# ehsan886/DBA_mod

Measured on AMD Instinct MI355X. Metric: FL rounds/sec + backdoor ASR & main-task acc, ResNet-18 CIFAR-10 100 clients, higher is better.
Workload: dtype fp32

## Files before the change

### csrc/kernels/xconv_fwd.hip

```cpp
#include "xhalo.hpp"

namespace xg {
SplitPolicy& split_policy() {
  static SplitPolicy p;
  return p;
}
}

namespace {

template <int W, int IMGS, int BN, int WM, int WN, bool PRE>
__global__ __launch_bounds__(256) void ximg_kernel(const XArgs a) {
  constexpr int P = 2, NT = 256;
  constexpr int PW = W + 2, PI = PW * PW, PP = IMGS * PI;
  constexpr int CC = 32, CH = CC / 8, Q4 = CC / 4;
  constexpr int PATCH = PP * CH;
  constexpr int BM = IMGS * W * W;
  constexpr int TM = BM / WM, TN = BN / WN, MI = TM / 32, NJ = TN / 32;
  static_assert(WM * WN == NT / 64 && MI >= 1 && NJ >= 1 && BM == 128, "tiling");
  constexpr int RPT = NT / 8;
  static_assert(BN % RPT == 0, "weight rows");
  constexpr int RB = BN / RPT, BPL = BN * 4;
  __shared__ __attribute__((aligned(16))) uint4 patch[P * PATCH];
  __shared__ __attribute__((aligned(16))) uint4 bring[2 * P * BPL];
// ... 76 lines not shown
#pragma unroll
  for (int i = 0; i < MI; ++i)
#pragma unroll
    for (int j = 0; j < NJ; ++j)
#pragma unroll
      for (int r = 0; r < 16; ++r) acc[i][j][r] = 0.f;

  int apix[MI], arow[MI];
#pragma unroll
  for (int i = 0; i < MI; ++i) {
    const int m = wm * TM + i * 32 + fr;
    const int im = m / (W * W), rem = m - im * (W * W);
    apix[i] = im * PI + (rem / W) * PW + rem % W;
    arow[i] = rem / W;
  }
  auto mma = [&](int t, int buf, int stn) __attribute__((always_inline)) {
    const int tap = t % 9, ti = tap / 3, tj = tap - ti * 3;
    const int toff = ti * PW + tj;
    const uint4* L = bring + buf * P * BPL;
    sfor<2>([&](auto KK) __attribute__((always_inline)) {
      const int ch = decltype(KK)::value * 2 + hf;
      uint4 af[P][MI], bfr[P][NJ];
#pragma unroll
      for (int i = 0; i < MI; ++i) {
        const int pp = apix[i] + toff;
        const int o = pp * CH + (ch ^ ((arow[i] + ti) & 3));
#pragma unroll
        for (int p = 0; p < P; ++p) af[p][i] = patch[p * PATCH + o];
      }
#pragma unroll
      for (int j = 0; j < NJ; ++j) {
        const int n = wn * TN + j * 32 + fr;
        const int o = n * 4 + (ch ^ ((n >> 2) & 3));
#pragma unroll
        for (int p = 0; p < P; ++p) bfr[p][j] = L[p * BPL + o];
      }
      mma_half<MI, NJ, P, true, RB, decltype(KK)::value>(af, bfr, acc, [&](int q) __attribute__((always_inline)) {
        lput_q(buf ^ 1, stn, q);
        gq(t + 3, stn, q);
      });
    });
  };
  auto step = [&](int t, int buf, int stn) __attribute__((always_inline)) {
    const int c = t / 9;
    mma(t, buf, stn);
    __syncthreads();
    if (t - 9 * c == 8 && c + 1 < NC) {
#pragma unroll
      for (int u = 0; u < NE; ++u) ppiece(u, hs.ma);
      if (c + 2 < NC) pload(c + 2);
      __syncthreads();
    }
  };

  hs.init(amax_read(a.amax_src, a.amax_src_ld, g), amax_read(a.amax_w, a.amax_w_ld, slot));
#pragma unroll
  for (int q = 0; q < RB; ++q) {
    gq(0, 0, q);
    gq(1, 1, q);
  }
  pload(0);
#pragma unroll
  for (int u = 0; u < NE; ++u) ppiece(u, hs.ma);
  if (NC > 1) pload(1);
#pragma unroll
  for (int q = 0; q < RB; ++q) {
    lput_q(0, 0, q);
    gq(2, 0, q);
  }
  __syncthreads();
  int t = 0;
  for (; t + 1 < NK; t += 2) {
    step(t, 0, 1);
    step(t + 1, 1, 0);
  }
  if (t < NK) step(t, 0, 1);
  hs.finish(acc);

  float* out = a.out + (long long)g * a.out_gstride;
  const float* bias = a.bias ? a.bias + (long long)slot * a.b_sstride : nullptr;
  const float* res = a.res ? a.res + (long long)g * a.out_gstride : nullptr;
  float vmax = 0.f;
#pragma unroll
  for (int j = 0; j < NJ; ++j) {
    const int n = n0 + wn * TN + j * 32 + fr;
    if (n >= a.Ncol) continue;
    const float bv = bias ? bias[n] : 0.f;
#pragma unroll
    for (int i = 0; i < MI; ++i)
#pragma unroll
      for (int r = 0; r < 16; ++r) {
        const int m = wm * TM + i * 32 + (r & 3) + 8 * (r >> 2) + 4 * hf;
        if (img0 + m / (W * W) >= nv) continue;
        const long long o = (long long)(img0 * W * W + m) * a.Ncol + n;
        float v = acc[i][j][r];
        if (bias) v += bv;
        if (res) v += res[o];
        if (a.relu) v = fmaxf(v, 0.f);
        vmax = fmaxf(vmax, fabsf(v));
        out[o] = v;
      }
  }
  if (a.amax_out) amax_fold(a.amax_out, a.amax_out_ld, g, vmax);
}

template <int W, int IMGS, int BN>
__global__ __launch_bounds__(256) void ximg2_kernel(const XArgs a) {
  constexpr int P = 2, NT = 256;
  constexpr int PW = W + 2, PI = PW * PW, PP = IMGS * PI;
  constexpr int CC = 32, CH = CC / 8, Q4 = CC / 4;
  constexpr int PATCH = PP * CH;
  constexpr int BM = IMGS * W * W;
  constexpr int WN = BN / 32, WM = (NT / 64) / WN, TM = BM / WM, MI = TM / 32;
  static_assert(WM * WN == NT / 64 && MI >= 1 && BM == 128, "tiling");
  extern __shared__ __attribute__((aligned(16))) uint4 ximg2_patch[];

  const int g = blockIdx.y;
  const int tn = blockIdx.x % a.tiles_n, tm = blockIdx.x / a.tiles_n;
  const int img0 = tm * IMGS, n0 = tn * BN;
  const int nv = min(valid_rows(a.nvalid, g, a.N), a.N);
  if (img0 >= nv) return;
  const int slot = a.wsel ? a.wsel[g] : g;
  const int Cs = a.Cs, NC = Cs / CC, NK = 9 * NC;
  const float* __restrict__ src = a.src + (long long)g * a.src_gstride;
  const int tid = threadIdx.x, lane = tid & 63, wid = tid >> 6;
  const int wm = wid / WN, wn = wid % WN;
  const int fr = lane & 31, hf = lane >> 5;

  constexpr int NE = (PP * Q4 + NT - 1) / NT;
  static_assert(NE <= 9, "one patch piece per k-step");
  float4 pv[NE];
  const __amdgpu_buffer_rsrc_t rA = rsrc(src, (long long)a.N * W * W * Cs * 4);
  auto pload1 = [&](int u, int cc) __attribute__((always_inline)) {
    const int e = tid + NT * u;
    const int pp = e / Q4, q = e - pp * Q4;
    const int im = pp / PI, rem = pp - im * PI;
    const int h = rem / PW - 1, w = rem % PW - 1, img = img0 + im;
    const bool ok = e < PP * Q4 && cc < NC && img < nv && (unsigned)h < (unsigned)W && (unsigned)w < (unsigned)W;
    pv[u] = bload4(rA, ok ? (((img * W + h) * W + w) * Cs + cc * CC + q * 4) * 4 : kOOB);
  };
  HScale hs;
  auto ppiece = [&](int u, int buf) __attribute__((always_inline)) {
    const int e = tid + NT * u;
    if (NT * (u + 1) > PP * Q4 && e >= PP * Q4) return;
    const int pp = e / Q4, q = e - pp * Q4;
    const int prow = (pp % PI) / PW;
    uint2 sp[P];
    split4h(pv[u].x, pv[u].y, pv[u].z, pv[u].w, hs.ma, sp);
    const int o = pp * CH + ((q >> 1) ^ (prow & 3));
#pragma unroll
    for (int p = 0; p < P; ++p) ((uint2*)&ximg2_patch[(buf * P + p) * PATCH + o])[q & 1] = sp[p];
  };

  const __amdgpu_buffer_rsrc_t rF = rsrc(a.wf + (long long)slot * a.wf_sstride, (long long)a.Ncol * 9 * Cs * 4);
  const int wbase = ((n0 >> 5) + wn) * NK * 4096 + lane * 16;
  uint4 wb[3][4];
  auto gw = [&](int t, int s, int f) __attribute__((always_inline)) {
    wb[s][f] = __builtin_bit_cast(uint4, bload4(rF, t < NK ? wbase + t * 4096 + f * 1024 : kOOB));
  };

  f32x16_t acc[MI][1];
#pragma unroll
  for (int i = 0; i < MI; ++i)
#pragma unroll
    for (int r = 0; r < 16; ++r) acc[i][0][r] = 0.f;

  int apix[MI], arow[MI];
#pragma unroll
  for (int i = 0; i < MI; ++i) {
    const int m = wm * TM + i * 32 + fr;
    const int im = m / (W * W), rem = m - im * (W * W);
    apix[i] = im * PI + (rem / W) * PW + rem % W;
    arow[i] = rem / W;
  }

  hs.init(amax_read(a.amax_src, a.amax_src_ld, g), amax_read(a.amax_w, a.amax_w_ld, slot));
#pragma unroll
  for (int f = 0; f < 4; ++f) {
    gw(0, 0, f);
    gw(1, 1, f);
  }
#pragma unroll
  for (int u = 0; u < NE; ++u) pload1(u, 0);
#pragma unroll
  for (int u = 0; u < NE; ++u) {
    ppiece(u, 0);
    pload1(u, 1);
  }
  __syncthreads();
  for (int c = 0; c < NC; ++c) {
    const uint4* L = ximg2_patch + (c & 1) * P * PATCH;
    const bool more = c + 1 < NC;
    sfor<9>([&](auto TAP) __attribute__((always_inline)) {
      constexpr int tap = decltype(TAP)::value, ti = tap / 3, tj = tap - ti * 3;
      constexpr int toff = ti * PW + tj, s = tap % 3, s2 = (tap + 2) % 3;
      constexpr int u = tap - (9 - NE);
      constexpr int NQ = u >= 0 ? 5 : 4;
      const int t = c * 9 + tap;
      __builtin_amdgcn_sched_barrier(0x786);
      sfor<2>([&](auto KK) __attribute__((always_inline)) {
        constexpr int kk = decltype(KK)::value;
        const int ch = kk * 2 + hf;
        uint4 af[P][MI], bfr[P][1];
#pragma unroll
        for (int i = 0; i < MI; ++i) {
          const int o = (apix[i] + toff) * CH + (ch ^ ((arow[i] + ti) & 3));
#pragma unroll
          for (int p = 0; p < P; ++p) af[p][i] = L[p * PATCH + o];
        }
#pragma unroll
        for (int p = 0; p < P; ++p) bfr[p][0] = wb[s][kk * 2 + p];
        mma_half<MI, 1, P, true, NQ, kk>(af, bfr, acc, [&](int q) __attribute__((always_inline)) {
          if (q < 4) {
            gw(t + 2, s2, q);
          } else if constexpr (u >= 0) {
            if (more) ppiece(u, (c + 1) & 1);
            pload1(u, c + 2);
          }
        });
      });
    });
    __syncthreads();
  }
  hs.finish(acc);

  float* out = a.out + (long long)g * a.out_gstride;
  const float* bias = a.bias ? a.bias + (long long)slot * a.b_sstride : nullptr;
  const float* res = a.res ? a.res + (long long)g * a.out_gstride : nullptr;
  float vmax = 0.f;
  const int n = n0 + wn * 32 + fr;
  if (n < a.Ncol) {
    const float bv = bias ? bias[n] : 0.f;
#pragma unroll
    for (int i = 0; i < MI; ++i)
#pragma unroll
      for (int r = 0; r < 16; ++r) {
        const int m = wm * TM + i * 32 + (r & 3) + 8 * (r >> 2) + 4 * hf;
        if (img0 + m / (W * W) >= nv) continue;
        const long long o = (long long)(img0 * W * W + m) * a.Ncol + n;
        float v = acc[i][0][r];
        if (bias) v += bv;
        if (res) v += res[o];
        if (a.relu) v = fmaxf(v, 0.f);
        vmax = fmaxf(vmax, fabsf(v));
        out[o] = v;
      }
  }
  if (a.amax_out) amax_fold(a.amax_out, a.amax_out_ld, g, vmax);
}

template <int W, int IMGS, int BN, int WM, int WN>
int ximg_go(const XArgs& a, int G, hipStream_t st) {
  XArgs b = a;
  b.tiles_n = ceil_div(a.Ncol, BN);
  const dim3 grid((unsigned)(ceil_div(a.N, IMGS) * b.tiles_n), G, 1);
  if (a.wp) hipLaunchKernelGGL((ximg_kernel<W, IMGS, BN, WM, WN, true>), grid, dim3(256), 0, st, b);
  else hipLaunchKernelGGL((ximg_kernel<W, IMGS, BN, WM, WN, false>), grid, dim3(256), 0, st, b);
  DBA_LAUNCH_CHECK();
}
template <int W, int IMGS, int BN>
int ximg2_go(const XArgs& a, int G, hipStream_t st) {
  constexpr int PATCH = IMGS * (W + 2) * (W + 2) * 4;
  constexpr int LDS = 2 * 2 * PATCH * (int)sizeof(uint4);
  static unsigned long long attr_set = 0ull;
  int dev = 0;
  if (hipGetDevice(&dev) != hipSuccess || dev < 0 || dev >= 64) return -100;
  if (!(attr_set >> dev & 1ull)) {
    if (hipFuncSetAttribute((const void*)ximg2_kernel<W, IMGS, BN>, hipFuncAttributeMaxDynamicSharedMemorySize,
                            LDS) != hipSuccess)
      return -100;
    attr_set |= 1ull << dev;
  }
  XArgs b = a;
  b.tiles_n = ceil_div(a.Ncol, BN);
  const dim3 grid((unsigned)(ceil_div(a.N, IMGS) * b.tiles_n), G, 1);
  hipLaunchKernelGGL((ximg2_kernel<W, IMGS, BN>), grid, dim3(256), LDS, st, b);
  DBA_LAUNCH_CHECK();
}
int& ximg_on() {
  static int on = 1;
  return on;
}
int ximg_try(const XArgs& a, int G, int KH, int KW, hipStream_t st) {
  const XClass& c = a.cls[0];
  if (!ximg_on() || KH != 3 || KW != 3 || a.sp != 1 || a.os != 1 || a.dsg != 1 || a.splitk != 1 || c.nI != 3 ||
      c.nJ != 3 || c.bh != -1 || c.bw != -1)
    return -100;
  if (a.Hs != a.Ho || a.Ws != a.Wo || a.Ho != a.Wo || a.Cs % 32 != 0 || a.Ncol % 32 != 0) return -100;
  if (a.bf.mode || a.lz_coef) return -100;
  if (!aligned16(a.src) || a.src_gstride % 4 || !aligned16(a.w) || a.w_sstride % 4) return -100;
  if (a.wp && (((uintptr_t)a.wp & 15) || a.wp_sstride % 8)) return -100;
  if (a.sc_src) return -100;
  if (ximg_on() == 1 && a.wp && a.wf && !((uintptr_t)a.wf & 15) && a.wf_sstride % 8 == 0) {
    int rc = -100;
    if (a.Wo == 8) rc = a.Ncol >= 128 ? ximg2_go<8, 2, 128>(a, G, st) : ximg2_go<8, 2, 64>(a, G, st);
    if (a.Wo == 4) rc = a.Ncol >= 128 ? ximg2_go<4, 8, 128>(a, G, st) : ximg2_go<4, 8, 64>(a, G, st);
    if (rc != -100) return rc;
  }
  if (a.Wo == 8) return a.Ncol >= 128 ? ximg_go<8, 2, 128, 2, 2>(a, G, st) : ximg_go<8, 2, 64, 2, 2>(a, G, st);
  if (a.Wo == 4) return a.Ncol >= 128 ? ximg_go<4, 8, 128, 2, 2>(a, G, st) : ximg_go<4, 8, 64, 2, 2>(a, G, st);
  return -100;
}

}

DBA_EXPORT int dba_xsplit_policy(int target, int min_k, int max_s, int kslab_max, int dgrad_ks) {
  SplitPolicy& p = split_policy();
  if (dgrad_ks >= 0) p.dgrad_ks = dgrad_ks;
  if (target > 0) p.target = target;
  if (min_k > 0) p.min_k = min_k;
  if (max_s > 0) p.max_s = std::min(max_s, kSkMax);
  if (kslab_max > 0) p.kslab_max = kslab_max;
  return 0;
}

DBA_EXPORT int dba_ximg_set(int on) {
  const int prev = ximg_on();
  if (on >= 0) ximg_on() = on;
  return prev;
}


DBA_EXPORT long long dba_xconv_ws_floats(int G, int N, int Ho, int Wo, int Cin, int Cout, int KH, int KW) {
  const long long M = (long long)N * Ho * Wo;
  const int s = xsplitk(M, G, Cout, KH * KW * Cin);
  return s > 1 ? (long long)s * G * M * Cout : 0;
}


DBA_EXPORT long long dba_xconv_sk_ints(int G, int N, int Ho, int Wo, int Cin, int Cout, int KH, int KW) {
  const long long M = (long long)N * Ho * Wo;
  const int s = xsplitk(M, G, Cout, KH * KW * Cin);
  const long long n = s > 1 ? xconv_sk_count(M, Cout, G, 1, s) : 0;
  return (n > 0 && sk_ok((const int*)1, n, M, Cout, G, 1, s)) ? n : 0;
}


DBA_EXPORT int dba_xconv_fwd(const float* x, long long x_gstride, const float* w, long long w_sstride,
                             const int* wsel, const float* bias, long long b_sstride, const float* res, float* out,
                             long long out_gstride, const int* nvalid, int G, int N, int H, int W, int Cin, int Ho,
                             int Wo, int Cout, int KH, int KW, int stride, int pad, int relu, const int* amax_x,
                             int amax_x_ld, const int* amax_w, int amax_w_ld, int* amax_out, int amax_out_ld,
                             const uint16_t* wp, long long wp_sstride, const uint16_t* wf, long long wf_sstride,
                             float* ws, long long ws_floats, int* sk_cnt,
                             long long sk_cnt_n, const void* bnf, const float* lz_coef, int lz_relu,
                             void* stream) {
  hipStream_t st = (hipStream_t)stream;
  if ((long long)N * H * W * Cin >= (1LL << 29)) return -103;
  const long long M = (long long)N * Ho * Wo;
  const int K = KH * KW * Cin;
  const int vec = (Cin % 4 == 0 && aligned16(x) && aligned16(w) && x_gstride % 4 == 0 && w_sstride % 4 == 0) ? 4 : 1;
  XArgs a{};
  a.src = x; a.src_gstride = x_gstride; a.w = w; a.w_sstride = w_sstride; a.wsel = wsel;
  a.bias = bias; a.b_sstride = b_sstride; a.res = res; a.out = out; a.out_gstride = out_gstride;
  a.nvalid = nvalid; a.N = N; a.Hs = H; a.Ws = W; a.Cs = Cin; a.Ncol = Cout; a.Ho = Ho; a.Wo = Wo;
  a.sp = stride; a.os = 1; a.dsg = 1; a.relu = relu; a.splitk = 1;
  a.amax_src = amax_x; a.amax_w = amax_w; a.amax_out = amax_out;
  a.amax_src_ld = amax_x_ld; a.amax_w_ld = amax_w_ld; a.amax_out_ld = amax_out_ld;
  a.wp = wp; a.wp_sstride = wp_sstride; a.wf = wf; a.wf_sstride = wf_sstride;
  a.cls[0] = XClass{KH, KW, -pad, -pad, 0, 0, Ho, Wo, 0};
  if (!amax_x || !amax_w) return -109;
  if (bnf) {
    a.bf = *(const BnFuse*)bnf;
    if (a.bf.mode != 1 || bias || res || relu || (Cout & 3) || a.bf.C != Cout) return -108;
  }
  if (lz_coef) {
    if (wp || vec < 4 || Cin > 512) return -108;
    a.lz_coef = lz_coef; a.lz_relu = lz_relu;
  }
  auto fin = [&](int rc) { return (rc == 0 && a.bf.mode) ? bnx_finalize_go(a.bf, nvalid, G, N, Ho * Wo, st) : rc; };
  if (stride == 1) {
    int rc = ximg_try(a, G, KH, KW, st);
    if (rc == -100) rc = xhalo_try(a, G, KH, KW, st);
    if (rc != -100) return fin(rc);
  }
  const int s = xsplitk(M, G, Cout, K);
  const bool ws_ok = s > 1 && ws != nullptr && ws_floats >= (long long)s * G * M * Cout;
  if (s > 1 && !(ws_ok && sk_ok(sk_cnt, sk_cnt_n, M, Cout, G, 1, s))) {
    XArgs b = a;
    b.kslab = s;
    const int rc = xconv_ks(b, M, G, vec, st);
    if (rc != -100) return fin(rc);
  }
  if (ws_ok && sk_ok(sk_cnt, sk_cnt_n, M, Cout, G, 1, s)) {
    XArgs b = a;
    b.splitk = s;
    b.zstride = (long long)G * M * Cout;
    b.sk_ws = ws; b.sk_gstride = M * Cout; b.sk_cnt = sk_cnt;
    return fin(xconv_dispatch(b, M, G, 1, vec, st));
  }
  if (ws_ok) {
    XArgs b = a;
    b.splitk = s;
    b.out = ws;
    b.out_gstride = M * Cout;
    b.zstride = (long long)G * M * Cout;
    const int rc = xconv_dispatch(b, M, G, 1, vec, st);
    if (rc != 0) return rc;
    if (a.bf.mode)
      return bnx_tile_go(a.bf, nullptr, out, out_gstride, nvalid, G, N, Ho * Wo, nullptr, 0.f, ws, s, b.zstride,
                         nullptr, st);
    const long long per = M * Cout;
    const dim3 grid((unsigned)std::max(1LL, std::min(1024LL, (per + 255) / 256)), G);
    hipLaunchKernelGGL(xsplitk_reduce_kernel, grid, dim3(256), 0, st, (const float*)ws, s, b.zstride, per, nvalid, N,
                       Ho * Wo, Cout, bias, b_sstride, wsel, res, relu, out, amax_out, amax_out_ld);
    DBA_LAUNCH_CHECK();
  }
  return fin(xconv_dispatch(a, M, G, 1, vec, st));
}


DBA_EXPORT int dba_xdown_fwd(const float* a_, long long a_gstride, const float* w2, long long w2_sstride,
                             const uint16_t* w2p, long long w2p_sstride, const int* wsel, const float* b2,
                             long long b_sstride, const float* x2, long long x2_gstride, const uint16_t* wscp,
                             long long wscp_sstride, const float* bsc, long long bsc_sstride, float* out,
                             long long out_gstride, const int* nvalid, int G, int N, int Ho, int Wo, int C, int H2,
                             int W2, int C2, const int* amax_a, int amax_a_ld, const int* amax_w2, int amax_w2_ld,
                             const int* amax_x2, int amax_x2_ld, const int* amax_wsc, int amax_wsc_ld, int* amax_out,
                             int amax_out_ld, void* stream) {
  if (!amax_a || !amax_w2 || !amax_x2 || !amax_wsc || !w2p || !wscp) return -109;
  if ((H2 - 1) / 2 + 1 != Ho || (W2 - 1) / 2 + 1 != Wo || (long long)N * H2 * W2 * C2 >= (1LL << 29) ||
      (long long)N * Ho * Wo * C >= (1LL << 29))
    return -103;
  XArgs a{};
  a.src = a_; a.src_gstride = a_gstride; a.w = w2; a.w_sstride = w2_sstride; a.wsel = wsel;
  a.bias = b2; a.b_sstride = b_sstride; a.res = nullptr; a.out = out; a.out_gstride = out_gstride;
  a.nvalid = nvalid; a.N = N; a.Hs = Ho; a.Ws = Wo; a.Cs = C; a.Ncol = C; a.Ho = Ho; a.Wo = Wo;
  a.sp = 1; a.os = 1; a.dsg = 1; a.relu = 1; a.splitk = 1;
  a.amax_src = amax_a; a.amax_w = amax_w2; a.amax_out = amax_out;
  a.amax_src_ld = amax_a_ld; a.amax_w_ld = amax_w2_ld; a.amax_out_ld = amax_out_ld;
  a.wp = w2p; a.wp_sstride = w2p_sstride;
  a.sc_src = x2; a.sc_gstride = x2_gstride; a.sc_H = H2; a.sc_W = W2; a.sc_C = C2;
  a.sc_wp = wscp; a.sc_wp_sstride = wscp_sstride;
  a.sc_amax_src = amax_x2; a.sc_amax_src_ld = amax_x2_ld; a.sc_amax_w = amax_wsc; a.sc_amax_w_ld = amax_wsc_ld;
  a.sc_bias = bsc; a.sc_b_sstride = bsc_sstride;
  a.cls[0] = XClass{3, 3, -1, -1, 0, 0, Ho, Wo, 0};
  return xhalo_try(a, G, 3, 3, (hipStream_t)stream);
}
```

### dba_mod_amd/ops/hip.py

```python
from __future__ import annotations

import contextlib
import ctypes
import os
from typing import Optional, Sequence, Tuple

import torch

from . import bnstate as bs
from . import build

Tensor = torch.Tensor
_F32 = torch.float32

if not os.path.exists(build.kernels_path()):
    raise ImportError(f"HIP kernel library missing: {build.kernels_path()} — run "
                      f"`python -m dba_mod_amd.ops.build` (or __graft_entry__.build())")
_L = ctypes.CDLL(build.kernels_path())

_P = ctypes.c_void_p
_I = ctypes.c_int
_LL = ctypes.c_longlong
_F = ctypes.c_float
_U = ctypes.c_uint
_D = ctypes.c_double

_SIGS = {
    "dba_gather_images": [_P, _P, _P, _P, _P, _P, _I, _P, _P, _I, _P, _I, _I, _I, _I, _I, _P],
    "dba_gather_rows": [_P, _P, _P, _P, _P, _I, _P, _P, _I, _P, _I, _P, _I, _I, _I, _P],
    "dba_xcolsum": [_P, _LL, _I, _P, _I, _I, _I, _P, _LL, _P, _P],
    "dba_xcolsum_part_doubles": [_I, _I, _I, _I],
    "dba_amax_segments": [_P, _LL, _P, _I, _I, _P, _I, _P],
    "dba_bn_fold": [_P, _LL, _P, _P, _P, _P, _P, _LL, _F, _P, _P, _I, _I, _I, _I, _P, _I, _P],
    "dba_relu_mask_bwd": [_P, _P, _P, _LL, _I, _P],
    "dba_maxpool": [_P, _P, _P, _LL, _I, _I, _I, _I, _I, _I, _I, _I, _I, _P],
    "dba_maxpool_bwd": [_P, _P, _P, _LL, _I, _I, _I, _I, _I, _I, _I, _I, _I, _P],
    "dba_avgpool": [_P, _P, _LL, _I, _I, _I, _P],
    "dba_avgpool_bwd": [_P, _P, _LL, _I, _I, _I, _P],
    "dba_dropout": [_P, _P, _I, _P, _U, _F, _LL, _I, _P],
    "dba_softmax_xent": [_P, _P, _I, _I, _I, _I, _P, _P, _P, _P, _LL, _P, _I, _P, _I, _P, _P, _P],
    "dba_softmax_xent_part_doubles": [_I, _I],
    "dba_xent_r5_set": [_I],
    "dba_head_train": [_P, _LL, _I, _I, _I, _I, _P, _LL, _P, _LL, _I, _P, _P, _P, _P, _P, _P, _LL, _P, _LL, _P, _P,
                       _P, _P, _LL, _P, _I, _I, _P],
    "dba_head_part_doubles": [_I, _I],
    "dba_sgd_step": [_P, _LL, _P, _P, _P, _P, _P, _F, _F, _P, _I, _I, _P],
    "dba_scale_from_base": [_P, _P, _F, _P, _LL, _P],
    "dba_add_noise_scaled": [_P, _P, _LL, _F, _F, _U, _I, _I, _P],
    "dba_delta_sum": [_P, _LL, _I, _P, _LL, _P, _P],
    "dba_sqdist_blocks": [_LL],
    "dba_gram_chunks": [_I],
    "dba_sq_dists": [_P, _LL, _P, _I, _LL, _P, _P, _P],
    "dba_weighted_sum": [_P, _LL, _P, _I, _P, _LL, _I, _P],
    "dba_weighted_sum_fixed": [_P, _LL, _P, _I, _P, _LL, _D, _P],
    "dba_gram": [_P, _LL, _I, _I, _P, _P, _P],
    "dba_delta_stats_blocks": [_LL],
    "dba_delta_stats": [_P, _LL, _I, _P, _LL, _P, _P, _P, _P, _P],
    "dba_clipped_delta_sum_fixed": [_P, _LL, _I, _P, _P, _P, _LL, _D, _P],
    "dba_clipped_delta_sum": [_P, _LL, _I, _P, _P, _P, _LL, _P],
    "dba_dist_loss_grad": [_P, _LL, _P, _LL, _P, _LL, _I, _P, _P, _F, _P, _P, _P],
    "dba_ximg_set": [_I],
    "dba_xwgrad_halo_set": [_I],
    "dba_xconv_ws_floats": [_I] * 8,
    "dba_xconv_fwd": [_P, _LL, _P, _LL, _P, _P, _LL, _P, _P, _LL, _P] + [_I] * 13 + [_P, _I] * 3 + [_P, _LL] * 3
    + [_P, _LL, _P, _P, _I, _P],
    "dba_xconv_sk_ints": [_I] * 8,
    "dba_xconv_dgrad": [_P, _LL, _P, _LL, _P, _P, _P, _LL, _P] + [_I] * 12 + [_P, _I] * 2 + [_P, _LL] * 3 + [_P, _P],
    "dba_xsplit_w": [_P, _LL, _LL, _I, _P, _I, _P, _P],
    "dba_amax": [_P, _LL, _LL, _P, _LL, _I, _P, _I, _P],
    "dba_xtranspose": [_P, _I, _I, _LL, _P, _P],
    "dba_xwgrad_ws_floats": [_I] * 8 + [_P],
    "dba_xwgrad_stem_ws_floats": [_I] * 6,
    "dba_xsplit_policy": [_I] * 5,
    "dba_xsplit_w_batch": [_P, _I, _I, _P],
    "dba_xfrag_w_batch": [_P, _I, _I, _P],
    "dba_bn_fold_batch": [_P, _I, _I, _F, _P],
    "dba_xwgrad": [_P, _LL, _P, _LL, _P, _LL, _P] + [_I] * 12 + [_P, _I] * 2 + [_P, _LL, _I] + [_P, _I, _P],
    "dba_bnx_rows": [_P, _P, _P, _LL, _P, _I, _I, _I, _P, _F, _P],
    "dba_bnx_apply": [_P, _P, _P, _P, _P, _I, _I, _P, _LL, _P, _I, _I, _I, _I, _P, _I, _P],
    "dba_bnfuse_size": [],
    "dba_xwgrad_stem": [_P, _LL, _P, _P, _P, _LL, _P, _P, _I, _I, _I, _I, _P],
    "dba_bnx_dy": [_P, _P, _P, _P, _LL, _P, _I, _I, _I, _I, _P, _I, _P],
    "dba_xwgrad_reduce_batch": [_P, _I, _I, _LL, _P],
    "dba_xblock_fwd": [_P, _LL, _P, _LL, _P, _P, _P, _LL, _P, _P, _LL, _P] + [_I] * 6
    + [_P, _I, _P, _P, _I, _P, _I, _P],
    "dba_xblock_stem_fwd": [_P, _LL, _P, _LL, _P, _P, _LL, _P, _LL, _P, _P, _LL, _P, _P, _LL, _P] + [_I] * 6
    + [_P, _P, _P, _I, _P, _I, _P],
    "dba_mlp_train": [_P, _I, _I, _I, _I, _I, _P, _LL, _P, _P, _I, _P, _I, _I, _I, _I, _P, _P, _P, _P, _I, _I,
                      _P, _LL, _I, _P, _F, _F, _P, _P],
    "dba_xdown_fwd": [_P, _LL, _P, _LL, _P, _LL, _P, _P, _LL, _P, _LL, _P, _LL, _P, _LL, _P, _LL, _P] + [_I] * 8
    + [_P, _I] * 5 + [_P],
    "dba_xstem_fwd": [_P, _LL, _P, _LL, _P, _P, _LL, _P, _P, _LL, _P] + [_I] * 13 + [_P, _I, _P, _P],
}
for _name, _args in _SIGS.items():
    _fn = getattr(_L, _name)
    _fn.argtypes = _args
    _fn.restype = ctypes.c_int
_L.dba_xconv_ws_floats.restype = ctypes.c_longlong
_L.dba_xconv_sk_ints.restype = ctypes.c_longlong
_L.dba_xwgrad_ws_floats.restype = ctypes.c_longlong
_L.dba_xwgrad_stem_ws_floats.restype = ctypes.c_longlong
_L.dba_xcolsum_part_doubles.restype = ctypes.c_longlong
_L.dba_softmax_xent_part_doubles.restype = ctypes.c_longlong
_L.dba_head_part_doubles.restype = ctypes.c_longlong


class _BnFuse(ctypes.Structure):
    _fields_ = [("mode", _I), ("C", _I), ("ngrp", _I),
                ("rec0", _P),
                ("coef_a", _P), ("gamma_a", _P), ("beta_a", _P), ("rm_a", _P), ("rv_a", _P),
                ("p_gstride", _LL), ("momentum", _F), ("eps", _F), ("relu", _I),
                ("amax_a", _P), ("amax_ld", _I),
                ("ya", _P), ("yb", _P), ("y_gstride", _LL),
                ("coef_b", _P), ("gamma_b", _P), ("amax_b", _P),
                ("dgamma_a", _P), ("dbeta_a", _P), ("dgamma_b", _P), ("dbeta_b", _P), ("gr_gstride", _LL),
                ("mask_out", _P), ("mask_lazy", _I)]


assert ctypes.sizeof(_BnFuse) == int(_L.dba_bnfuse_size()), "BnFuse layout mismatch (rebuild the kernels)"


NOT_HANDLED = -100
F16_PAIR = 16


def _call(name: str, *args) -> int:
    rc = getattr(_L, name)(*args)
    if rc != 0 and rc != NOT_HANDLED:
        raise RuntimeError(f"{name}: HIP error {rc}")
    return rc


def _ptr(t: Optional[Tensor]):
    return None if t is None else t.data_ptr()


def _stream():
    return torch.cuda.current_stream().cuda_stream


def _i32(t: Optional[Tensor]) -> Optional[Tensor]:
    if t is None:
        return None
    return t if (t.dtype == torch.int32 and t.is_contiguous()) else t.to(torch.int32).contiguous()


def _inner_contig(t: Tensor) -> bool:
    exp = 1
    for d in range(t.dim() - 1, 0, -1):
        if t.shape[d] != 1 and t.stride(d) != exp:
            return False
        exp *= t.shape[d]
    return True


def _rowview(t: Tensor) -> Tuple[Tensor, int]:
    if not _inner_contig(t):
        t = t.contiguous()
    return t, (t.stride(0) if t.shape[0] > 1 else int(torch.tensor(t.shape[1:]).prod()))


def _act(t: Tensor, dt: Optional[torch.dtype] = None, what: str = "activation") -> Tensor:
    if t.dtype != _F32:
        raise TypeError(f"{what}: unsupported dtype {t.dtype} (fp32 only)")
    if dt is not None and t.dtype != dt:
        raise TypeError(f"{what}: dtype {t.dtype} does not match the op's {dt} operands "
                        f"(no silent precision conversion)")
    return t.contiguous()


def _f32(t: Tensor) -> int:
    return int(t.dtype == _F32)


_UNIT_AMAX = {}


def _unit_amax(G: int, device):
    key = (G, device)
    if key not in _UNIT_AMAX:
        a = torch.zeros(AMAX_SUB, _amax_ld(G), dtype=torch.int32, device=device)
        a[0, :G] = 0x3F800000
        _UNIT_AMAX[key] = a
    return _UNIT_AMAX[key]


def gather_images(src, labels, idx, trig_masks, trig_id, poison_n, target, flip_seeds, out_dtype):
    G, B = idx.shape
    _, H, W, C = src.shape
    x = torch.empty(G, B, H, W, C, dtype=out_dtype, device=src.device)
    y = torch.empty(G, B, dtype=torch.int32, device=src.device)
    idx, trig_id, poison_n, fs = _i32(idx), _i32(trig_id), _i32(poison_n), _i32(flip_seeds)
    _call("dba_gather_images", src.data_ptr(), _i32(labels).data_ptr(), idx.data_ptr(),
          trig_masks.contiguous().data_ptr(), trig_id.data_ptr(), poison_n.data_ptr(), int(target), _ptr(fs),
          x.data_ptr(), int(out_dtype == torch.float32), y.data_ptr(), G, B, H, W, C, _stream())
    if out_dtype == _F32:
        x._dba_amax = _unit_amax(G, x.device)
    return x, y


def gather_rows(src, labels, idx, trig_cols, trig_vals, trig_id, poison_n, target, out_dtype):
    G, B = idx.shape
    Fd = src.shape[1]
    x = torch.empty(G, B, Fd, dtype=out_dtype, device=src.device)
    y = torch.empty(G, B, dtype=torch.int32, device=src.device)
    tc = _i32(trig_cols)
    _call("dba_gather_rows", src.contiguous().data_ptr(), _i32(labels).data_ptr(), _i32(idx).data_ptr(),
          tc.data_ptr(), trig_vals.float().contiguous().data_ptr(), int(tc.shape[1]), _i32(trig_id).data_ptr(),
          _i32(poison_n).data_ptr(), int(target), x.data_ptr(), int(out_dtype == torch.float32), y.data_ptr(),
          G, B, Fd, _stream())
    return x, y


_MLP_LAYERS = ("layer1.0.weight", "layer1.0.bias", "layer2.0.weight", "layer2.0.bias", "layer3.0.weight",
               "layer3.0.bias")


def mlp_train(spec, sched, t0, t1, B, state, mom, fg, rows, labels, trig_cols, trig_vals, target, stats,
              max_slots, nan_flag, momentum, wd, prof=None) -> int:
    G = state.shape[0]
    es = [spec.by_name[n] for n in _MLP_LAYERS]
    offs = torch.tensor([e.offset for e in es], dtype=torch.int32)
    (H1, F), (H2, _), (C, _) = es[0].k_shape[:2], es[2].k_shape[:2], es[4].k_shape[:2]
    assert sched.dtype == torch.int32 and sched.is_contiguous() and state.stride(1) == 1
    tc = _i32(trig_cols)
    return _call("dba_mlp_train", sched.data_ptr(), sched.shape[1], int(t0), int(t1), G, B, state.data_ptr(),
                 state.stride(0), mom.data_ptr(), _ptr(fg), spec.P, offs.data_ptr(), F, H1, H2, C,
                 rows.contiguous().data_ptr(), _i32(labels).data_ptr(), tc.data_ptr(),
                 trig_vals.float().contiguous().data_ptr(), int(tc.shape[1]), int(target), stats.data_ptr(),
                 stats.shape[1], max_slots, nan_flag.data_ptr(), float(momentum), float(wd), _ptr(prof), _stream())


def _check_w(w: Tensor, dt: torch.dtype = _F32) -> Tuple[Tensor, int]:
    if w.dtype != dt:
        raise TypeError(f"conv weights: dtype {w.dtype} does not match the {dt} activations "
                        f"(no silent precision conversion)")
    return _rowview(w)


def set_ximg(on: int) -> int:
    return int(_L.dba_ximg_set(int(on)))


def set_wgrad_halo(on: int) -> int:
    return int(_L.dba_xwgrad_halo_set(int(on)))


def set_split_policy(target: int = -1, min_k: int = -1, max_s: int = -1, kslab_max: int = -1,
                     dgrad_ks: int = -1) -> None:
    _call("dba_xsplit_policy", int(target), int(min_k), int(max_s), int(kslab_max), int(dgrad_ks))


_STEM_WGRAD = True


def set_stem_wgrad(on: int) -> int:
    global _STEM_WGRAD
    prev = int(_STEM_WGRAD)
    if on >= 0:
        _STEM_WGRAD = bool(on)
    return prev


def fp32_mode() -> int:
    return F16_PAIR


AMAX_SUB = 16


def _amax_ld(G: int) -> int:
    return max(32, (G + 31) // 32 * 32)


class _AmaxArena:

    def __init__(self, G: int, device, n: int, counters: int = 0) -> None:
        self.G, self.ld, self.next = G, _amax_ld(G), 0
        slots = n * AMAX_SUB * self.ld
        flat = torch.zeros(slots + counters, dtype=torch.int32, device=device)
        self.buf = flat[:slots].view(n, AMAX_SUB, self.ld)
        self.cnt, self.cnt_next = flat[slots:], 0

    def counters(self, n: int, device):
        if n <= 0 or device != self.cnt.device or self.cnt_next + n > self.cnt.numel():
            return None
        self.cnt_next += n
        return self.cnt[self.cnt_next - n:self.cnt_next]

    def take(self, G: int, device):
        if G != self.G or self.next >= self.buf.shape[0] or device != self.buf.device:
            return None
        self.next += 1
        return self.buf[self.next - 1]


_ARENA: list = []


@contextlib.contextmanager
def amax_arena(G: int, device, n: int = 256, counters: int = 0):
    _ARENA.append(_AmaxArena(G, device, n, counters))
    try:
        yield
    finally:
        _ARENA.pop()


def amax_slots(n: int, G: int, device):
    return torch.zeros(n, AMAX_SUB, _amax_ld(G), dtype=torch.int32, device=device)


def _amax_new(G: int, device):
    a = _ARENA[-1].take(G, device) if _ARENA else None
    return a if a is not None else torch.zeros(AMAX_SUB, _amax_ld(G), dtype=torch.int32, device=device)


def _sk_counters(n: int, device):
    if n <= 0 or not _ARENA:
        return None
    return _ARENA[-1].counters(n, device)


def _aptr(a):
    return (None, 0) if a is None else (a.data_ptr(), a.shape[-1])


def _amax(t, gstride, n_per_g, nvalid=None, per_item=0):
    G = t.shape[0]
    out = _amax_new(G, t.device)
    _call("dba_amax", t.data_ptr(), gstride, n_per_g, _ptr(_i32(nvalid)), per_item, G, out.data_ptr(), out.shape[1],
          _stream())
    return out


def _amax_out(t):
    if t.dtype != _F32:
        return None
    a = _amax_new(t.shape[0], t.device)
    t._dba_amax = a
    return a


def weight_amax(flat, segments):
    G, n = flat.shape[0], len(segments)
    ar = _ARENA[-1] if _ARENA else None
    if ar is not None and ar.G == G and ar.buf.device == flat.device and ar.next + n <= ar.buf.shape[0]:
        buf, ar.next = ar.buf[ar.next:ar.next + n], ar.next + n
    else:
        buf = torch.zeros(n, AMAX_SUB, _amax_ld(G), dtype=torch.int32, device=flat.device)
    slots, base = list(buf), buf.data_ptr()
    d = torch.tensor(segments, dtype=torch.int64)
    _call("dba_amax_segments", flat.data_ptr(), flat.stride(0), d.data_ptr(), len(segments), G, base,
          slots[0].shape[1], _stream())
    return slots


def split_weights(w, sstride: int, per: int, amax):
    slots = w.shape[0]
    out = torch.empty(slots, 2, per, dtype=torch.int16, device=w.device)
    _call("dba_xsplit_w", w.data_ptr(), sstride, per, slots, amax.data_ptr(), amax.shape[1], out.data_ptr(), _stream())
    w._dba_planes = out
    frag_weights_batch([w])
    return out


def split_weights_batch(items) -> None:
    if not items:
        return
    slots = items[0][0].shape[0]
    desc, outs = [], []
    for w, sstride, per, amax in items:
        assert w.shape[0] == slots and w.dtype == torch.float32
        out = torch.empty(slots, 2, per, dtype=torch.int16, device=w.device)
        desc.append([w.data_ptr(), sstride, per, amax.data_ptr(), amax.shape[1], out.data_ptr(), 0])
        outs.append(out)
    d = torch.tensor(desc, dtype=torch.int64)
    _call("dba_xsplit_w_batch", d.data_ptr(), len(items), slots, _stream())
    for (w, *_), out in zip(items, outs):
        w._dba_planes = out
    frag_weights_batch([w for w, *_ in items])


def frag_weights_batch(ws) -> None:
    desc, outs = [], []
    for w in ws:
        p = getattr(w, "_dba_planes", None)
        if (p is None or w.dim() != 5 or tuple(w.shape[2:4]) != (3, 3) or w.shape[1] % 32 or w.shape[4] % 32
                or not p.is_contiguous() or p.shape[2] != w[0].numel()):
            continue
        out = torch.empty(p.shape[0], 2 * p.shape[2], dtype=torch.int16, device=p.device)
        desc.append([p.data_ptr(), out.data_ptr(), w.shape[1], w.shape[4], 0])
        outs.append((w, out))
    if not desc:
        return
    d = torch.tensor(desc, dtype=torch.int64)
    _call("dba_xfrag_w_batch", d.data_ptr(), len(desc), outs[0][1].shape[0], _stream())
    for w, out in outs:
        w._dba_fplanes = out


def _wplanes(w):
    p = getattr(w, "_dba_planes", None)
    return (None, 0) if p is None else (p.data_ptr(), p.stride(0))


def _wfplanes(w):
    p = getattr(w, "_dba_fplanes", None)
    return (None, 0) if p is None else (p.data_ptr(), p.stride(0))


def _amax_w(w, gstride, n):
    a = getattr(w, "_dba_amax", None)
    if a is None:
        a = _amax(w, gstride, n)
        w._dba_amax = a
    return a


def _amax_act(t, nvalid):
    a = getattr(t, "_dba_amax", None)
    if a is not None:
        return a
    per_item = t[0, 0].numel()
    a = _amax(t, t.stride(0), t.shape[1] * per_item, nvalid, per_item)
    t._dba_amax = a
    return a


_EVAL_STEM_MFMA = os.environ.get("DBA_EVAL_STEM7_MFMA", "1") != "0"
_EVAL_STEM_PAD = True


def _xconv_fwd(x, w, wsel, stride, pad, bias, residual, relu, nvalid, out_dtype, bnf=None, lz=None):
    if out_dtype not in (None, _F32):
        raise TypeError(f"fp32 conv cannot emit {out_dtype} (no silent precision conversion)")
    G, N, H, W, Cin = x.shape
    attrs = {k: getattr(w, k) for k in ("_dba_amax", "_dba_planes", "_dba_fplanes") if hasattr(w, k)}
    w, ws = _check_w(w, _F32)
    for k, v in attrs.items():
        setattr(w, k, v)
    Cout, KH, KW = w.shape[1], w.shape[2], w.shape[3]
    assert w.shape[4] == Cin, (w.shape, x.shape)
    Ho = (H + 2 * pad - KH) // stride + 1
    Wo = (W + 2 * pad - KW) // stride + 1
    y = torch.empty(G, N, Ho, Wo, Cout, dtype=_F32, device=x.device)
    bs = 0
    if bias is not None:
        if bias.dtype != _F32:
            raise TypeError(f"conv bias must be fp32 (got {bias.dtype})")
        bias, bs = _rowview(bias)
    res = _act(residual, _F32, "residual") if residual is not None else None
    ay = _amax_out(y) if bnf is None else None
    bnf_p = ctypes.byref(bnf) if bnf is not None else None
    eval_mfma = (_EVAL_STEM_MFMA and "_dba_planes" in attrs and bnf is None and KH * KW * Cin > 64)
    if eval_mfma and Cin % 4 and _EVAL_STEM_PAD and lz is None:
        cp = 4 - Cin % 4
        x4 = torch.nn.functional.pad(x, (0, cp))
        x4._dba_amax = _amax_act(x, nvalid)
        w4 = torch.nn.functional.pad(w, (0, cp)).contiguous()
        per4 = w4[0].numel()
        a4 = attrs.get("_dba_amax")
        split_weights(w4, per4, per4, a4 if a4 is not None else _amax_w(w4, per4, per4))
        if a4 is not None:
            w4._dba_amax = a4
        return _xconv_fwd(x4, w4, wsel, stride, pad, bias, residual, relu, nvalid, out_dtype)
    if Cin <= 4 and not eval_mfma:
        rc = _call("dba_xstem_fwd", x.data_ptr(), N * H * W * Cin, w.data_ptr(), ws, _ptr(_i32(wsel)), _ptr(bias), bs,
                   _ptr(res), y.data_ptr(), N * Ho * Wo * Cout, _ptr(_i32(nvalid)), G, N, H, W, Cin, Ho, Wo, Cout,
                   KH, KW, stride, pad, int(relu), *_aptr(ay), bnf_p, _stream())
        if rc != NOT_HANDLED:
            return y
    n = int(_L.dba_xconv_ws_floats(G, N, Ho, Wo, Cin, Cout, KH, KW))
    wsb = torch.empty(n, dtype=_F32, device=x.device) if n > 0 else None
    ncnt = int(_L.dba_xconv_sk_ints(G, N, Ho, Wo, Cin, Cout, KH, KW)) if n > 0 else 0
    cnt = _sk_counters(ncnt, x.device)
    ax = lz[2] if lz is not None else _amax_act(x, nvalid)
    aw = _amax_w(w, ws, Cout * KH * KW * Cin)
    lz_coef, lz_relu = (lz[0].data_ptr(), int(lz[1])) if lz is not None else (None, 0)
    _call("dba_xconv_fwd", x.data_ptr(), N * H * W * Cin, w.data_ptr(), ws, _ptr(_i32(wsel)), _ptr(bias), bs,
          _ptr(res), y.data_ptr(), N * Ho * Wo * Cout, _ptr(_i32(nvalid)), G, N, H, W, Cin, Ho, Wo, Cout, KH, KW,
          stride, pad, int(relu), *_aptr(ax), *_aptr(aw), *_aptr(ay), *_wplanes(w), *_wfplanes(w), _ptr(wsb), n,
          _ptr(cnt), 0 if cnt is None else cnt.numel(), bnf_p, lz_coef, lz_relu, _stream())
    return y


_EVAL_BLOCK = os.environ.get("DBA_EVAL_BLOCK", "1") != "0"
_BLOCK_SHAPES = {(32, 32)}


def basic_block_ok(x, w1, w2) -> bool:
    if not (_EVAL_BLOCK and x.dtype == _F32 and x.dim() == 5):
        return False
    H, W, C = x.shape[2:]
    return (H == W and (W, C) in _BLOCK_SHAPES
            and all(w.dtype == _F32 and tuple(w.shape[1:]) == (C, 3, 3, C)
                    and getattr(w, "_dba_planes", None) is not None for w in (w1, w2)))


def basic_block_eval(x, w1, b1, w2, b2, wsel=None, nvalid=None):
    x = _act(x, _F32, "conv input")
    G, N, _, W, C = x.shape
    per = C * 9 * C
    (w1c, ws1), (w2c, ws2) = _check_w(w1), _check_w(w2)
    aw1, aw2 = _amax_w(w1, ws1, per), _amax_w(w2, ws2, per)
    p1, p2 = w1._dba_planes, w2._dba_planes
    assert p1.stride(0) == p2.stride(0) and aw1.shape[1] == aw2.shape[1]
    (b1c, bs1), (b2c, bs2) = _rowview(b1), _rowview(b2)
    assert bs1 == bs2 and b1c.dtype == b2c.dtype == _F32
    ax = _amax_act(x, nvalid)
    y = torch.empty_like(x)
    ay = _amax_out(y)
    rc = _call("dba_xblock_fwd", x.data_ptr(), x.stride(0), y.data_ptr(), y.stride(0), _ptr(_i32(wsel)),
               p1.data_ptr(), p2.data_ptr(), p1.stride(0), b1c.data_ptr(), b2c.data_ptr(), bs1, _ptr(_i32(nvalid)),
               G, N, W, W, C, C, *_aptr(ax), aw1.data_ptr(), aw2.data_ptr(), aw1.shape[1], *_aptr(ay), _stream())
    if rc == NOT_HANDLED:
        raise RuntimeError("xblock_fwd declined a shape basic_block_ok accepted")
    return y


_EVAL_STEM = os.environ.get("DBA_EVAL_STEM", "1") != "0"


def stem_block_ok(x, w0, w1, w2) -> bool:
    if not (_EVAL_STEM and _EVAL_BLOCK and x.dtype == _F32 and x.dim() == 5 and tuple(x.shape[2:]) == (32, 32, 3)):
        return False
    return (w0.dtype == _F32 and tuple(w0.shape[1:]) == (32, 3, 3, 3) and getattr(w0, "_dba_planes", None) is not None
            and all(w.dtype == _F32 and tuple(w.shape[1:]) == (32, 3, 3, 32)
                    and getattr(w, "_dba_planes", None) is not None for w in (w1, w2)))


def stem_block_eval(x, w0, b0, w1, b1, w2, b2, wsel=None, nvalid=None):
    x = _act(x, _F32, "image")
    G, N, _, W, Ci = x.shape
    C = w1.shape[1]
    per = C * 9 * C
    (w0c, ws0), (w1c, ws1), (w2c, ws2) = _check_w(w0), _check_w(w1), _check_w(w2)
    aw0 = _amax_w(w0, ws0, C * 9 * Ci)
    aw1, aw2 = _amax_w(w1, ws1, per), _amax_w(w2, ws2, per)
    p0, p1, p2 = w0._dba_planes, w1._dba_planes, w2._dba_planes
    assert p1.stride(0) == p2.stride(0) and aw0.shape[1] == aw1.shape[1] == aw2.shape[1]
    (b0c, bs0), (b1c, bs1), (b2c, bs2) = _rowview(b0), _rowview(b1), _rowview(b2)
    assert bs1 == bs2 and b0c.dtype == b1c.dtype == b2c.dtype == _F32
    y = torch.empty(G, N, W, W, C, dtype=_F32, device=x.device)
# ... 647 lines not shown
```

Measured before the change: 3.565.

## Add specialized stride-2 3x3 conv forward kernel with parity-split LDS patch

Adds a dedicated forward kernel for stride-2 3x3 convolutions, dispatched ahead of the generic path. It stages an input row-band into LDS split by row and column parity, so each tap reads contiguous fragments, and it keeps a rolling register ring of weight fragments interleaved with the MFMA ops. It is only enabled for 16x16 output with 32 input channels (the ResNet-18 layer2 downsample conv) and can be toggled from Python. The aim is to replace the generic split-k/im2col path for that layer, at the cost of more specialised code and dynamic LDS setup.

```diff
diff --git a/csrc/kernels/xconv_fwd.hip b/csrc/kernels/xconv_fwd.hip
--- a/csrc/kernels/xconv_fwd.hip
+++ b/csrc/kernels/xconv_fwd.hip
@@ -402,6 +402,178 @@
   return -100;
 }
 
+template <int WO, int R, int BN>
+__global__ __launch_bounds__(256, 4) void xs2_kernel(const XArgs a) {
+  constexpr int P = 2, NT = 256, WI = 2 * WO, RT = WO / R;
+  constexpr int PP = (2 * R + 1) * WI;
+  constexpr int SB1 = (R + 1) * WO, SA1 = 2 * SB1;
+  constexpr int HP = PP + 1, HB = 2 * HP;
+  constexpr int BM = R * WO;
+  constexpr int WN = BN / 32, WM = (NT / 64) / WN, TM = BM / WM, MI = TM / 32, PER = 3 * MI;
+  constexpr int NE = (PP * 8 + NT - 1) / NT;
+  constexpr int RS = 6, WD = 5;
+  static_assert(WM * WN == NT / 64 && MI >= 1 && TM % 32 == 0 && RT * R == WO && NE <= 9, "tiling");
+  extern __shared__ __attribute__((aligned(16))) uint4 xs2_patch[];
+
+  const int g = blockIdx.y;
+  const int tn = blockIdx.x % a.tiles_n, tm = blockIdx.x / a.tiles_n;
+  const int img = tm / RT, r0 = (tm % RT) * R, n0 = tn * BN;
+  const int nv = min(valid_rows(a.nvalid, g, a.N), a.N);
+  if (img >= nv) return;
+  const int slot = a.wsel ? a.wsel[g] : g;
+  const int Cs = a.Cs, NK = 9;
+  const float* __restrict__ src = a.src + (long long)g * a.src_gstride;
+  const int tid = threadIdx.x, lane = tid & 63, wid = tid >> 6;
+  const int wm = wid / WN, wn = wid % WN;
+  const int fr = lane & 31, hf = lane >> 5;
+
+  float4 pv[NE];
+  const __amdgpu_buffer_rsrc_t rA = rsrc(src, (long long)a.N * WI * WI * Cs * 4);
+  auto pload1 = [&](int u) __attribute__((always_inline)) {
+    const int e = tid + NT * u;
+    const int pp = e >> 3, q = e & 7;
+    const int h = 2 * r0 - 1 + pp / WI, w = pp % WI;
+    const bool ok = e < PP * 8 && (unsigned)h < (unsigned)WI;
+    pv[u] = bload4(rA, ok ? (((img * WI + h) * WI + w) * Cs + q * 4) * 4 : kOOB);
+  };
+  HScale hs;
+  auto ppiece = [&](int u) __attribute__((always_inline)) {
+    const int e = tid + NT * u;
+    if (NT * (u + 1) > PP * 8 && e >= PP * 8) return;
+    const int pp = e >> 3, q = e & 7;
+    const int pr = pp / WI, w = pp % WI;
+    const int loc = ((pr & 1) ? SA1 + (w & 1) * R * WO : (w & 1) * SB1) + (pr >> 1) * WO + (w >> 1);
+    uint2 sp[P];
+    split4h(pv[u].x, pv[u].y, pv[u].z, pv[u].w, hs.ma, sp);
+#pragma unroll
+    for (int p = 0; p < P; ++p) ((uint2*)&xs2_patch[(((q >> 2) * P + p) * 2 + ((q >> 1) & 1)) * HP + loc])[q & 1] = sp[p];
+  };
+
+  const __amdgpu_buffer_rsrc_t rF = rsrc(a.wf + (long long)slot * a.wf_sstride, (long long)a.Ncol * 9 * Cs * 4);
+  const int wbase = ((n0 >> 5) + wn) * NK * 4096 + lane * 16;
+  uint4 wb[RS][P];
+  auto gw = [&](int t, int kk, int s, int p) __attribute__((always_inline)) {
+    wb[s][p] = __builtin_bit_cast(uint4, bload4(rF, t < NK ? wbase + t * 4096 + (kk * 2 + p) * 1024 : kOOB));
+  };
+
+  f32x16_t acc[MI][1];
+#pragma unroll
+  for (int i = 0; i < MI; ++i)
+#pragma unroll
+    for (int r = 0; r < 16; ++r) acc[i][0][r] = 0.f;
+
+  int abase[MI];
+  bool acol0[MI];
+#pragma unroll
+  for (int i = 0; i < MI; ++i) {
+    const int m = wm * TM + i * 32 + fr;
+    abase[i] = hf * HP + m;
+    acol0[i] = m % WO == 0;
+  }
+  const int azero = hf * HP + PP;
+  auto hstep = [&](auto TAP, auto S, auto NQC, const uint4* L, auto&& fill) __attribute__((always_inline)) {
+    constexpr int tap = decltype(TAP)::value, s = decltype(S)::value, NQ = decltype(NQC)::value;
+    constexpr int ti = tap / 3, tj = tap - ti * 3;
+    constexpr int tc = ((ti & 1) ? SA1 + (tj != 1) * R * WO : (tj != 1) * SB1) + (ti >> 1) * WO - (tj == 0);
+    __builtin_amdgcn_sched_barrier(0x786);
+    uint4 af[P][MI];
+#pragma unroll
+    for (int i = 0; i < MI; ++i) {
+      int o = abase[i] + tc;
+      if (tj == 0) o = acol0[i] ? azero : o;
+#pragma unroll
+      for (int p = 0; p < P; ++p) af[p][i] = L[p * HB + o];
+    }
+    sfor<PER>([&](auto C) __attribute__((always_inline)) {
+      constexpr int c = decltype(C)::value, p = c / MI, i = c % MI;
+      acc[i][0] = mfma16<true>(af[prod_pa(P, p)][i], wb[s][prod_pb(P, p)], acc[i][0]);
+      sfor<NQ>([&](auto Q) __attribute__((always_inline)) {
+        constexpr int q = decltype(Q)::value;
+        if constexpr ((c + 1) * NQ >= (q + 1) * PER && c * NQ < (q + 1) * PER) fill(q);
+      });
+    });
+  };
+
+  hs.init(amax_read(a.amax_src, a.amax_src_ld, g), amax_read(a.amax_w, a.amax_w_ld, slot));
+  if (tid < 4 * P) xs2_patch[tid * HP + PP] = make_uint4(0u, 0u, 0u, 0u);
+#pragma unroll
+  for (int hq = 0; hq < WD; ++hq)
+#pragma unroll
+    for (int p = 0; p < P; ++p) gw(hq >> 1, hq & 1, hq, p);
+#pragma unroll
+  for (int u = 0; u < NE; ++u) pload1(u);
+#pragma unroll
+  for (int u = 0; u < NE; ++u) ppiece(u);
+  __syncthreads();
+  sfor<18>([&](auto HQ) __attribute__((always_inline)) {
+    constexpr int hq = decltype(HQ)::value, h2 = hq + WD;
+    hstep(std::integral_constant<int, hq / 2>{}, std::integral_constant<int, hq % RS>{},
+          std::integral_constant<int, 2>{}, xs2_patch + (hq & 1) * P * HB, [&](int q) __attribute__((always_inline)) {
+            gw(h2 >> 1, h2 & 1, h2 % RS, q);
+          });
+  });
+  hs.finish(acc);
+
+  float* out = a.out + (long long)g * a.out_gstride;
+  const float* bias = a.bias ? a.bias + (long long)slot * a.b_sstride : nullptr;
+  const float* res = a.res ? a.res + (long long)g * a.out_gstride : nullptr;
+  float vmax = 0.f;
+  const int n = n0 + wn * 32 + fr;
+  if (n < a.Ncol) {
+    const float bv = bias ? bias[n] : 0.f;
+#pragma unroll
+    for (int i = 0; i < MI; ++i)
+#pragma unroll
+      for (int r = 0; r < 16; ++r) {
+        const int m = wm * TM + i * 32 + (r & 3) + 8 * (r >> 2) + 4 * hf;
+        const long long o = (long long)((img * WO + r0) * WO + m) * a.Ncol + n;
+        float v = acc[i][0][r];
+        if (bias) v += bv;
+        if (res) v += res[o];
+        if (a.relu) v = fmaxf(v, 0.f);
+        vmax = fmaxf(vmax, fabsf(v));
+        out[o] = v;
+      }
+  }
+  if (a.amax_out) amax_fold(a.amax_out, a.amax_out_ld, g, vmax);
+}
+
+template <int WO, int R, int BN>
+int xs2_go(const XArgs& a, int G, hipStream_t st) {
+  constexpr int LDS = 2 * 2 * ((2 * R + 1) * 2 * WO + 1) * 2 * (int)sizeof(uint4);
+  static unsigned long long attr_set = 0ull;
+  int dev = 0;
+  if (hipGetDevice(&dev) != hipSuccess || dev < 0 || dev >= 64) return -100;
+  if (!(attr_set >> dev & 1ull)) {
+    if (hipFuncSetAttribute((const void*)xs2_kernel<WO, R, BN>, hipFuncAttributeMaxDynamicSharedMemorySize,
+                            LDS) != hipSuccess)
+      return -100;
+    attr_set |= 1ull << dev;
+  }
+  XArgs b = a;
+  b.tiles_n = ceil_div(a.Ncol, BN);
+  const dim3 grid((unsigned)(a.N * (WO / R) * b.tiles_n), G, 1);
+  hipLaunchKernelGGL((xs2_kernel<WO, R, BN>), grid, dim3(256), LDS, st, b);
+  DBA_LAUNCH_CHECK();
+}
+int& xs2_on() {
+  static int on = 1;
+  return on;
+}
+int xs2_try(const XArgs& a, int G, int KH, int KW, hipStream_t st) {
+  const XClass& c = a.cls[0];
+  if (!xs2_on() || KH != 3 || KW != 3 || a.sp != 2 || a.os != 1 || a.dsg != 1 || a.splitk != 1 || c.nI != 3 ||
+      c.nJ != 3 || c.bh != -1 || c.bw != -1)
+    return -100;
+  if (a.Hs != a.Ws || (a.Ws & 1) || a.Ho != a.Hs / 2 || a.Wo != a.Ws / 2 || a.Cs % 32 != 0 || a.Ncol % 32 != 0)
+    return -100;
+  if (a.bf.mode || a.lz_coef || a.sc_src) return -100;
+  if (!aligned16(a.src) || a.src_gstride % 4) return -100;
+  if (!a.wf || ((uintptr_t)a.wf & 15) || a.wf_sstride % 8) return -100;
+  if (a.Wo == 16 && a.Cs == 32) return xs2_go<16, 4, 64>(a, G, st);
+  return -100;
+}
+
 }
 
 DBA_EXPORT int dba_xsplit_policy(int target, int min_k, int max_s, int kslab_max, int dgrad_ks) {
@@ -417,6 +589,13 @@
 DBA_EXPORT int dba_ximg_set(int on) {
   const int prev = ximg_on();
   if (on >= 0) ximg_on() = on;
+  return prev;
+}
+
+
+DBA_EXPORT int dba_xs2_set(int on) {
+  const int prev = xs2_on();
+  if (on >= 0) xs2_on() = on;
   return prev;
 }
 
@@ -474,6 +653,10 @@
     if (rc == -100) rc = xhalo_try(a, G, KH, KW, st);
     if (rc != -100) return fin(rc);
   }
+  if (stride == 2) {
+    const int rc = xs2_try(a, G, KH, KW, st);
+    if (rc != -100) return fin(rc);
+  }
   const int s = xsplitk(M, G, Cout, K);
   const bool ws_ok = s > 1 && ws != nullptr && ws_floats >= (long long)s * G * M * Cout;
   if (s > 1 && !(ws_ok && sk_ok(sk_cnt, sk_cnt_n, M, Cout, G, 1, s))) {
diff --git a/dba_mod_amd/ops/hip.py b/dba_mod_amd/ops/hip.py
--- a/dba_mod_amd/ops/hip.py
+++ b/dba_mod_amd/ops/hip.py
@@ -60,6 +60,7 @@
     "dba_clipped_delta_sum": [_P, _LL, _I, _P, _P, _P, _LL, _P],
     "dba_dist_loss_grad": [_P, _LL, _P, _LL, _P, _LL, _I, _P, _P, _F, _P, _P, _P],
     "dba_ximg_set": [_I],
+    "dba_xs2_set": [_I],
     "dba_xwgrad_halo_set": [_I],
     "dba_xconv_ws_floats": [_I] * 8,
     "dba_xconv_fwd": [_P, _LL, _P, _LL, _P, _P, _LL, _P, _P, _LL, _P] + [_I] * 13 + [_P, _I] * 3 + [_P, _LL] * 3
@@ -240,6 +241,10 @@
 
 def set_ximg(on: int) -> int:
     return int(_L.dba_ximg_set(int(on)))
+
+
+def set_xs2(on: int) -> int:
+    return int(_L.dba_xs2_set(int(on)))
 
 
 def set_wgrad_halo(on: int) -> int:
```

Result: no change. 3.588 (median of 6 runs) (+0.7%).
